# big-nacho/patolette

Measured on AMD Instinct MI355X. Metric: Mpixels/sec quantized (256-color ICtCp + KMeans) at 1 GPU; palette ΔE vs ref, higher is better.
Workload: dtype f64

## Files before the change

patolette_amd/csrc/pipeline.hip:

```cpp
#include <algorithm>
#include <functional>
#include <chrono>
#include <cmath>
#include <atomic>
#include <memory>
#include <mutex>
#include <thread>
#include <future>

#include "color_device.h"
#include "common.h"
#include "host_math.h"
#include "kmeans.h"
#include "map.h"
#include "saliency.h"
#include "quant.h"
#include "rgba.h"
#include "compact.h"

namespace pamd {

void launch_convert(int which, const double *src, double *dst, size_t n, ConvertStats *stats, hipStream_t s, BinK sumk = BinK{0.0, 0.0},
                    BinK momk = BinK{0.0, 0.0}, size_t begin = 0, size_t end = ~(size_t)0, bool init_stats = true);
void launch_convert_rows(int which, const double *rows, double *dst, size_t n, ConvertStats *stats, hipStream_t s,
// ... 124 lines not shown
    while (hi - lo > 1) { const int mid = (lo + hi) >> 1; if (t0[mid] <= t) lo = mid; else hi = mid; }
    return lo;
}
__global__ __launch_bounds__(256) void k_round_setup(NodeDev *table, RoundSetup a) {
    const size_t tid = (size_t)blockIdx.x * blockDim.x + threadIdx.x, stride = (size_t)gridDim.x * blockDim.x;
    for (size_t i = tid; i < (size_t)a.nr; i += stride) {
        const NodeIn in = a.recs[i];
        NodeDev &d = table[a.ids[i]];
        d.begin = in.begin; d.n = in.n; d.gn = in.gn; d.buf = in.buf; d.slot = in.slot; d.child0 = in.child0; d.nchild = in.nchild;
        for (int j = 0; j < 3; j++) { d.axis[j] = in.axis[j]; d.mean[j] = in.mean[j]; }
        d.sw = in.sw; d.klin = in.klin; d.kquad = in.kquad;
    }
    for (size_t i = tid; i < (size_t)a.nr * kNodeResetElems; i += stride)
        node_reset_element(table[a.ids[i / kNodeResetElems]], (int)(i % kNodeResetElems));
    for (size_t t = tid; t < (size_t)a.ntA; t += stride) {
        const int r = node_of_tile(a.tA0, a.nr, (int)t);
        const unsigned long long o = (unsigned long long)((int)t - a.tA0[r]) * kTileA, n = a.recs[r].n;
        a.tilesA[t] = Tile{a.recs[r].begin + o, (unsigned)(n - o < (unsigned long long)kTileA ? n - o : kTileA), (unsigned)a.ids[r]};
    }
    for (size_t t = tid; t < (size_t)a.ntP; t += stride) {
        const int r = node_of_tile(a.tP0, a.nr, (int)t);
        const unsigned long long o = (unsigned long long)((int)t - a.tP0[r]) * kTileP, n = a.recs[r].n;
        a.tilesP[t] = Tile{a.recs[r].begin + o, (unsigned)(n - o < (unsigned long long)kTileP ? n - o : kTileP), (unsigned)a.ids[r]};
    }
    for (size_t i = tid; i < a.nhist; i += stride) a.hist[i] = 0.0;
    for (size_t i = tid; i < a.nbk; i += stride) { a.hsize[i] = 0ULL; a.hcount[i] = 0u; }
}


struct GqOut { int kbase, error, pad[2]; int cuts[16]; unsigned long long ticks[8]; };

constexpr int kLqDevMaxK = 256;
constexpr int kLqNodeCap = 16 * kLqDevMaxK + 256;
constexpr int kLqRoundCap = 512;
constexpr int kLqMaxRounds = 96;

struct LqRec {
    double val;
    int left;
    int kn;
};
struct LqCen { double mean[3]; double gn; };
struct LqHead {
    int done, error, rounds, nnodes, neval, pad;
    unsigned long long split_evals, split_px;
    double tau;
    double round_px[kLqMaxRounds], round_nr[kLqMaxRounds];
};
struct LqCtl {
    LqHead h;
    int K, M, nleaves, pad;
    int ncids[2];
    RoundDyn dyn;
    int leaves[kLqNodeCap];
    int round_ids[kLqRoundCap];
    int cids[2][2 * kLqRoundCap];
    int tA0[kLqRoundCap + 1], tP0[kLqRoundCap + 1];
    int nparent[kLqNodeCap];
    double np[kLqNodeCap];
    LqRec nrec[kLqNodeCap];
    LqCen ncen[kLqNodeCap];
};
template <> struct WsPoison<LqCtl> {
    static void dev(LqCtl *p, size_t a, size_t b) {
        for (size_t i = a; i < b; i++) {
            char *c = reinterpret_cast<char *>(p + i);
            ws_poison_dev(c + offsetof(LqCtl, h) + offsetof(LqHead, tau), sizeof(double) * (1 + 2 * kLqMaxRounds));
            ws_poison_dev(c + offsetof(LqCtl, np), sizeof(LqCtl::np));
            ws_poison_dev_rows(c + offsetof(LqCtl, nrec), sizeof(LqRec), sizeof(double), kLqNodeCap);
            ws_poison_dev(c + offsetof(LqCtl, ncen), sizeof(LqCtl::ncen));
        }
    }
    static void host(LqCtl *, size_t, size_t) {}
};

template <int CTRL, int ROW_MASK>
__device__ __forceinline__ double dpp_max_f64(const double v) {
    const int lo = __double2loint(v), hi = __double2hiint(v);
    const int tlo = __builtin_amdgcn_update_dpp(lo, lo, CTRL, ROW_MASK, 0xf, false);
    const int thi = __builtin_amdgcn_update_dpp(hi, hi, CTRL, ROW_MASK, 0xf, false);
    return fmax(v, __hiloint2double(thi, tlo));
}

__global__ __launch_bounds__(256) void k_lq_children(NodeDev *nodes, LqCtl *c, const int call, int init_kbase,
                                                     const int init_first, int init_nnodes, const int init_K, const GqOut *gq) {
    const bool init = init_kbase > 0;
    if (!init && c->h.done) return;
    if (init && gq) { init_kbase = gq->kbase; init_nnodes = init_first + init_kbase; }
    const int ncids = init ? init_kbase : c->ncids[call & 1];
    const int wave = (int)blockIdx.x * 4 + (int)(threadIdx.x >> 6), lane = threadIdx.x & 63;
    if (init && blockIdx.x == 0 && threadIdx.x == 0) {
        c->K = init_K; c->M = init_K - init_kbase; c->nleaves = 0; c->ncids[0] = init_kbase; c->dyn = RoundDyn{0, 0, 0, 0};
        c->h.done = 0; c->h.error = 0; c->h.rounds = 0; c->h.nnodes = init_nnodes; c->h.neval = 0; c->h.split_evals = 0ULL; c->h.split_px = 0ULL;
        c->h.tau = 0.0;
        for (int r = 0; r < kLqMaxRounds; r++) { c->h.round_px[r] = 0.0; c->h.round_nr[r] = 0.0; }
        if (gq && gq->error) { c->h.done = 1; c->h.error = 3; c->ncids[0] = 0; }
        for (int i = 0; i < init_first; i++) { c->nrec[i] = LqRec{0.0, -1, 1}; c->np[i] = 0.0; c->nparent[i] = -1; }
    }
    if (init && gq && gq->error) return;
    if (wave >= ncids) return;
    const int id = init ? init_first + wave : c->cids[call & 1][wave];
    if (init && lane == 0) c->cids[0][wave] = id;
    NodeDev &d = nodes[id];
    const double *acc = &d.acc[0][0][0];
    double sum = 0;
    if (lane < 14) {
        double v[kSlots];
#pragma unroll
        for (int k = 0; k < kSlots; k++) v[k] = acc[k * 14 + lane];
#pragma unroll
        for (int k = 0; k < kSlots; k++) sum += v[k];
    }
    const double pair = sum + __shfl_down(sum, 1, 64);
    double cov[7];
#pragma unroll
    for (int q = 0; q < 7; q++)
        cov[q] = __hiloint2double(__builtin_amdgcn_readlane(__double2hiint(pair), 2 * q), __builtin_amdgcn_readlane(__double2loint(pair), 2 * q));
    if (lane != 0) return;
    double ub = cov[6];
    const bool single = d.gn <= 1ULL;
    const double sw = d.sw;
    if (single || !(sw > 0)) ub = 0;
    else {
        double c6[6];
        for (int q = 0; q < 6; q++) c6[q] = cov[q] / sw;
        const double b = hm::lambda_max_bound(c6) * sw * (1.0 + 1e-9) + 1e-9 * cov[6];
        if (b == b && b < ub) ub = b;
    }
    for (int q = 0; q < 6; q++) d.cov6[q] = cov[q];
    d.dist = cov[6]; d.ub = ub; d.axis_state = 0;
    c->nrec[id] = LqRec{single ? 0.0 : ub, -1, single ? 1 : 0};
    c->nparent[id] = init ? -1 : c->round_ids[wave >> 1];
    c->ncen[id] = LqCen{{d.mean[0], d.mean[1], d.mean[2]}, (double)d.gn};
    c->leaves[(init ? 0 : c->nleaves) + wave] = id;
}

__device__ __forceinline__ int block_excl_scan_256(const int v, int *sw , int &total) {
    const int lane = threadIdx.x & 63, wid = threadIdx.x >> 6;
    const int inc = (int)wave_scan_incl_u32((unsigned)v);
    __syncthreads();
    if (lane == 63) sw[wid] = inc;
    __syncthreads();
    int base = 0;
    for (int w = 0; w < wid; w++) base += sw[w];
    total = sw[0] + sw[1] + sw[2] + sw[3];
    return base + inc - v;
}

__device__ __forceinline__ unsigned long long lq_key(const double p) { return p > 0.0 ? (unsigned long long)__double_as_longlong(p) : 0ULL; }

constexpr double kSpecBeta = 0.25;

__global__ __launch_bounds__(256) void k_lq_select(NodeDev *nodes, LqCtl *c, const int call, const int e_lin, const int e_quad) {
    if (c->h.done) return;
    const int tid = threadIdx.x, lane = tid & 63;
    const int cur = call & 1, nxt = cur ^ 1;
    const int ncids = c->ncids[cur];
    if (blockIdx.x > 0) {
        const int w = ((int)blockIdx.x - 1) * 4 + (tid >> 6);
        if (w >= ncids) return;
        NodeDev &d = nodes[c->cids[cur][w]];
        if (d.gn <= 1ULL || !(d.sw > 0)) { if (lane == 0) d.axis_state = d.gn <= 1ULL ? 0 : -1; return; }
        double c6[6];
        for (int q = 0; q < 6; q++) c6[q] = d.cov6[q] / d.sw;
        double a[9] = {c6[0], c6[1], c6[2], c6[1], c6[3], c6[4], c6[2], c6[4], c6[5]};
        double wv[3];
        const int info = hm::eigen_sym3(a, wv);
        if (lane == 0) {
            if (info != 0) d.axis_state = -1;
            else { d.axis[0] = a[6]; d.axis[1] = a[7]; d.axis[2] = a[8]; d.axis_state = 1; }
        }
        return;
    }
    __shared__ int sw[5];
    __shared__ unsigned int hist[256];
    __shared__ unsigned long long s_prefix, s_px;
    __shared__ int s_need, s_neval, s_first;
    __shared__ double s_umax[4];
    const int M = c->M;
    const int nn = c->h.nnodes;
    const int nr_prev = c->dyn.nr;
    int evald = 0;
    for (int i = tid; i < nr_prev; i += 256) {
        const int id = c->round_ids[i];
        const NodeDev &d = nodes[id];
        if (d.axis_state < 0) { c->nrec[id] = LqRec{0.0, -1, 1}; c->np[id] = 0.0; continue; }
        const int l = d.child0;
        const double b = d.dist - (nodes[l].dist + nodes[l + 1].dist);
        const int par = c->nparent[id];
        const double pp = par < 0 ? INFINITY : c->np[par];
        c->nrec[id].val = b; c->nrec[id].kn = 1;
        c->np[id] = b < pp ? b : pp;
        evald++;
    }
    if (tid == 0) { s_neval = 0; s_px = 0ULL; }
    __syncthreads();
    if (evald) atomicAdd(&s_neval, evald);
    __syncthreads();
    const int neval = c->h.neval + s_neval;
    double tau = 0.0;
    if (neval >= M && M > 0) {
        unsigned long long prefix = 0ULL;
        int need = M;
        for (int pass = 0; pass < 3; pass++) {
            const int shift = 56 - 8 * pass;
            hist[tid] = 0u;
            __syncthreads();
            for (int i = tid; i < nn; i += 256) {
                const LqRec r = c->nrec[i];
                if (r.kn && r.left >= 0) {
                    const unsigned long long k = lq_key(c->np[i]);
                    if (pass == 0 || (k >> (shift + 8)) == (prefix >> (shift + 8))) atomicAdd(&hist[(k >> shift) & 255ULL], 1u);
                }
            }
            __syncthreads();
            {
                const int mine = (int)hist[255 - tid];
                int total;
                const int excl = block_excl_scan_256(mine, sw, total);
                if (tid == 0) s_first = 256;
                __syncthreads();
                if (excl + mine >= need && tid <= 254) atomicMin(&s_first, tid);
                __syncthreads();
                const int f = s_first;
                if (f < 256) { if (tid == f) { s_need = need - excl; s_prefix = prefix | ((unsigned long long)(255 - f) << shift); } }
                else if (tid == 254) { s_need = need - (excl + mine); s_prefix = prefix; }
            }
            __syncthreads();
            need = s_need; prefix = s_prefix;
        }
        tau = __longlong_as_double((long long)prefix);
    }
    const double thr = fmax(kDelta, tau * (1.0 - 1e-9));
    const int nleaves = c->nleaves + ncids;
    auto leaf_prio = [&](const int id) -> double {
        const LqRec r = c->nrec[id];
        const int par = c->nparent[id];
        if (r.kn || (par >= 0 && nodes[par].axis_state < 0)) return -1.0;
        const double pp = par < 0 ? INFINITY : c->np[par];
        return r.val < pp ? r.val : pp;
    };
    double thr2 = thr;
    if (c->h.rounds < 48) {
        double u = -1.0;
        for (int i = tid; i < nleaves; i += 256) { const double pr = leaf_prio(c->leaves[i]); u = pr > u ? pr : u; }
#pragma unroll
        for (int o = 32; o > 0; o >>= 1) { const double v = __shfl_xor(u, o, 64); u = v > u ? v : u; }
        __syncthreads();
        if (lane == 0) s_umax[tid >> 6] = u;
        __syncthreads();
        u = fmax(fmax(s_umax[0], s_umax[1]), fmax(s_umax[2], s_umax[3]));
        if (kSpecBeta * u > thr2) thr2 = kSpecBeta * u;
    }
    int nkeep = 0, nr = 0;
    for (int base = 0; base < nleaves; base += 256) {
        const int i = base + tid;
        int id = -1, sel = 0, keep = 0;
        if (i < nleaves) {
            id = c->leaves[i];
            const double pr = leaf_prio(id);
            sel = pr >= thr2 ? 1 : 0;
            keep = (!sel && pr >= thr) ? 1 : 0;
        }
        int tsel, tkeep;
        const int psel = block_excl_scan_256(sel, sw, tsel);
        if (nr + tsel > kLqRoundCap && sel && nr + psel >= kLqRoundCap) { sel = 0; keep = 1; }
        const int pkeep = block_excl_scan_256(keep, sw, tkeep);
        if (sel) c->round_ids[nr + psel] = id;
        __syncthreads();
        if (keep) c->leaves[nkeep + pkeep] = id;
        nr = min(nr + tsel, kLqRoundCap);
        nkeep += tkeep;
        __syncthreads();
    }
    if (nr == 0) {
        if (tid == 0) { c->h.done = 1; c->h.neval = neval; c->h.tau = tau; c->nleaves = 0; c->ncids[nxt] = 0; c->dyn = RoundDyn{0, 0, 0, 0}; }
        return;
    }
    if (nn + 2 * nr > kLqNodeCap) {
        if (tid == 0) { c->h.done = 1; c->h.error = 2; c->dyn = RoundDyn{0, 0, 0, 0}; }
        return;
    }
    int runA = 0, runP = 0;
    for (int base = 0; base < nr; base += 256) {
        const int r = base + tid;
        int ta = 0, tp = 0;
        unsigned long long n = 0ULL;
        if (r < nr) {
            const int id = c->round_ids[r];
            NodeDev &d = nodes[id];
            d.slot = r; d.child0 = nn + 2 * r; d.nchild = 2;
            int P = 1;
            while ((1ULL << P) < (d.gn > 1ULL ? d.gn : 2ULL)) P++;
            d.klin = make_bink(e_lin, P); d.kquad = make_bink(e_quad, P);
            c->nrec[id].left = nn + 2 * r;
            c->cids[nxt][2 * r] = nn + 2 * r; c->cids[nxt][2 * r + 1] = nn + 2 * r + 1;
            n = d.n;
            ta = (int)((n + kTileA - 1) / kTileA); tp = (int)((n + kTileP - 1) / kTileP);
        }
        int totA, totP;
        const int pa = block_excl_scan_256(ta, sw, totA);
        const int pp = block_excl_scan_256(tp, sw, totP);
        if (r < nr) { c->tA0[r] = runA + pa; c->tP0[r] = runP + pp; }
        runA += totA; runP += totP;
        for (int o = 32; o > 0; o >>= 1) n += __shfl_xor(n, o, 64);
        if (lane == 0 && n) atomicAdd(&s_px, n);
    }
    __syncthreads();
    if (tid == 0) {
        const int round = c->h.rounds;
        const unsigned long long rpx = s_px;
        c->tA0[nr] = runA; c->tP0[nr] = runP;
        c->nleaves = nkeep; c->ncids[nxt] = 2 * nr;
        c->dyn = RoundDyn{nr, runA, runP, 0};
        c->h.nnodes = nn + 2 * nr; c->h.neval = neval; c->h.tau = tau;
        c->h.split_evals += (unsigned long long)nr; c->h.split_px += rpx; c->h.rounds = round + 1;
        if (round < kLqMaxRounds) { c->h.round_px[round] = (double)rpx; c->h.round_nr[round] = (double)nr; }
    }
}

__global__ __launch_bounds__(256) void k_lq_export(const LqCtl *c, LqHead *head, LqRec *rec, LqCen *cen) {
    const int nn = c->h.nnodes;
    const int t = blockIdx.x * blockDim.x + threadIdx.x, stride = gridDim.x * blockDim.x;
    for (int i = t; i < nn; i += stride) { rec[i] = c->nrec[i]; cen[i] = c->ncen[i]; }
    const double *src = reinterpret_cast<const double *>(&c->h);
    double *dst = reinterpret_cast<double *>(head);
    for (int i = t; i < (int)(sizeof(LqHead) / sizeof(double)); i += stride) dst[i] = src[i];
}

struct LqCommit { int row, node, new_row, left; };
__global__ void k_lq_trace(const NodeDev *nodes, const LqCommit *commits, int n, patolette_amd__SplitRecord *out) {
    const int t = blockIdx.x * blockDim.x + threadIdx.x;
    if (t >= n) return;
    const LqCommit cm = commits[t];
    const NodeDev &h = nodes[cm.node], &hl = nodes[cm.left], &hr = nodes[cm.left + 1];
    patolette_amd__SplitRecord tr;
    tr.row = cm.row; tr.new_row = cm.new_row;
    tr.split = hl.psplit < 0 ? -1 : (hl.psplit & 0xffff); tr.degenerate = hl.psplit < 0 ? 0 : (hl.psplit >> 16) & 1;
    tr.n = h.gn; tr.n_left = hl.gn; tr.n_right = hr.gn; tr.sw = h.sw;
    for (int j = 0; j < 3; j++) tr.axis[j] = h.axis[j];
    for (int q = 0; q < 6; q++) tr.cov6[q] = h.cov6[q] / h.sw;
    tr.dist = h.dist; tr.dist_left = hl.dist; tr.dist_right = hr.dist; tr.benefit = h.dist - (hl.dist + hr.dist);
    out[t] = tr;
}

__global__ __launch_bounds__(256) void k_round_setup_dyn(NodeDev *table, const LqCtl *c, Tile *tilesA, Tile *tilesP, double *hist,
                                                         unsigned long long *hsize, unsigned int *hcount, const size_t lqs) {
    const int nr = c->dyn.nr;
    if (nr == 0) return;
    const int ntA = c->dyn.ntA, ntP = c->dyn.ntP;
    const size_t tid = (size_t)blockIdx.x * blockDim.x + threadIdx.x, stride = (size_t)gridDim.x * blockDim.x;
    for (size_t i = tid; i < (size_t)nr * kNodeResetElems; i += stride)
        node_reset_element(table[c->round_ids[i / kNodeResetElems]], (int)(i % kNodeResetElems));
    for (size_t t = tid; t < (size_t)ntA; t += stride) {
        const int r = node_of_tile(c->tA0, nr, (int)t);
        const NodeDev &d = table[c->round_ids[r]];
        const unsigned long long o = (unsigned long long)((int)t - c->tA0[r]) * kTileA, n = d.n;
        tilesA[t] = Tile{d.begin + o, (unsigned)(n - o < (unsigned long long)kTileA ? n - o : kTileA), (unsigned)c->round_ids[r]};
    }
    for (size_t t = tid; t < (size_t)ntP; t += stride) {
        const int r = node_of_tile(c->tP0, nr, (int)t);
        const NodeDev &d = table[c->round_ids[r]];
        const unsigned long long o = (unsigned long long)((int)t - c->tP0[r]) * kTileP, n = d.n;
        tilesP[t] = Tile{d.begin + o, (unsigned)(n - o < (unsigned long long)kTileP ? n - o : kTileP), (unsigned)c->round_ids[r]};
    }
    for (size_t i = tid; i < lqs * (size_t)nr; i += stride) hist[i] = 0.0;
    for (size_t i = tid; i < (size_t)nr * kBuckets; i += stride) { hsize[i] = 0ULL; hcount[i] = 0u; }
}

struct GqTab {
    unsigned long long w0[kBuckets + 1];
    double t[10][kBuckets + 9];
    __device__ double distortion(int a, int b) const {
        if (w0[a] == w0[b]) return 0;
        const double q0 = t[0][b] - t[0][a], q1 = t[1][b] - t[1][a], q2 = t[2][b] - t[2][a];
        return t[3][b] - t[3][a] - (q0 * q0 + q1 * q1 + q2 * q2) / (double)(w0[b] - w0[a]);
    }
    __device__ double vcov(int a, int b, int r, int s) const {
        if (w0[a] == w0[b]) return 0;
        const double cnt = (double)(w0[b] - w0[a]);
        const int rs = 4 + s * (s + 1) / 2 + r;
        return (t[rs][b] - t[rs][a]) / cnt - (t[r][b] - t[r][a]) * (t[s][b] - t[s][a]) / (cnt * cnt);
    }
    __device__ bool axis(int a, int b, double ax[3]) const {
        double m[9] = {0, 0, 0, 0, 0, 0, 0, 0, 0};
        for (int s = 0; s < 3; s++) for (int r = 0; r <= s; r++) m[s * 3 + r] = vcov(a, b, r, s);
        m[0 * 3 + 2] = m[2 * 3 + 0]; m[0 * 3 + 1] = m[1 * 3 + 0]; m[1 * 3 + 2] = m[2 * 3 + 1];
        double w[3];
        if (hm::eigen_sym3(m, w) != 0) return false;
        ax[0] = m[6]; ax[1] = m[7]; ax[2] = m[8];
        return true;
    }
    __device__ static double norm3(const double a[3]) { double s = 0; for (int i = 0; i < 3; i++) s += a[i] * a[i]; return sqrt(s); }
    __device__ double bias(int a, int b, const double ax[3]) const {
        double ca[3];
        if (!axis(a, b, ca)) return -1;
        const double norms = norm3(ax) * norm3(ca);
        if (norms < 1e-16) return 0;
        const double dot = (ca[0] * ax[0] + ca[1] * ax[1] + ca[2] * ax[2]);
        return fmin(1.0, fabs(dot / norms));
    }
};

__device__ __forceinline__ void gq_dp_entry(const GqTab &c, const double *Ep, const int k, const int n, const int lane, double &e_out, int &cut_out) {
    double best = INFINITY; int bt = -1;
    for (int t = n - 2 - lane; t >= k - 1; t -= 64) {
        const double v = Ep[t] + c.distortion(t, n);
        if (v < best) { best = v; bt = t; }
    }
#pragma unroll
    for (int o = 32; o > 0; o >>= 1) {
        const double v2 = __shfl_down(best, o, 64); const int t2 = __shfl_down(bt, o, 64);
        if (t2 >= 0 && (bt < 0 || v2 < best || (v2 == best && t2 > bt))) { best = v2; bt = t2; }
    }
    double e = Ep[n - 1]; int cut = n - 1;
    if (bt >= 0 && best < e) { e = best; cut = bt; }
    e_out = e; cut_out = cut;
}

__global__ __launch_bounds__(1024) void k_gq_control(const double *__restrict__ hist, const unsigned int *__restrict__ hcount, GqDpDev *g,
                                                     const int palette_size, const int weighted, NodeDev *nodes, const int base0,
                                                     unsigned char *lut, GqOut *out, GqOut *out_host) {
    __shared__ GqTab c;
    __shared__ double E[2][kBuckets + 1];
    __shared__ int s_q[16], s_nq, s_stop, s_err, s_top;
    __shared__ double s_ax[3], s_cd[16], s_cb[16];
    __shared__ unsigned char s_lut[kBuckets];
    __shared__ double s_part[kGqMaxK][4][2];
    __shared__ unsigned long long s_cnt[kGqMaxK];
    const int tid = threadIdx.x, lane = tid & 63, wv = tid >> 6;
    __shared__ unsigned long long s_ticks[8];
    if (tid == 0) { for (int i = 0; i < 8; i++) s_ticks[i] = 0; s_ticks[0] = wall_clock64(); }
    for (int i = tid; i < 10 * kBuckets; i += 1024) {
        const int hq = i / kBuckets, b = i - hq * kBuckets;
        c.t[hq][b + 1] = hist[(size_t)(hq * 2 + 0) * kBuckets + b] + hist[(size_t)(hq * 2 + 1) * kBuckets + b];
    }
    for (int b = tid; b < kBuckets; b += 1024) c.w0[b + 1] = hcount[b];
    if (tid < 10) c.t[tid][0] = 0;
    if (tid == 10) c.w0[0] = 0;
    __syncthreads();
    if (tid == 0) s_ticks[5] = wall_clock64();
    if (wv < 10) {
        double *t = c.t[wv];
        double v[8];
#pragma unroll
        for (int u = 0; u < 8; u++) v[u] = t[1 + lane * 8 + u];
        double carry = 0, cin = 0;
        for (int l = 0; l < 64; l++) {
            double a = carry;
#pragma unroll
// ... 200 lines not shown
    if (i >= n) return;
    NodeDev &d = table[ids[i]];
    for (int q = 0; q < 7; q++) {
        for (int k = 1; k < kSlots; k++) { d.acc[k][q][0] = 0; d.acc[k][q][1] = 0; }
        d.acc[0][q][0] = buf[(size_t)i * 14 + 2 * q]; d.acc[0][q][1] = buf[(size_t)i * 14 + 2 * q + 1];
    }
}
__global__ void k_shard_children_local(NodeDev *table, const int *round_nodes, int nround) {
    const int i = blockIdx.x * blockDim.x + threadIdx.x;
    if (i >= nround) return;
    const NodeDev &nd = table[round_nodes[i]];
    for (int k = 0; k < nd.nchild; k++) {
        NodeDev &ch = table[nd.child0 + k];
        ch.begin = nd.cbegin[k]; ch.n = nd.cbegin[k + 1] - nd.cbegin[k];
    }
}

struct Bounds {
    double cmax, range, wmax; int e_lin, e_quad; double lo[3], hi[3];
    bool have_sum = false; double sum[3] = {0, 0, 0};
    bool have_mom = false;
    double sum2[3][2] = {{0, 0}, {0, 0}, {0, 0}}, mom2[6][2] = {{0, 0}, {0, 0}, {0, 0}, {0, 0}, {0, 0}, {0, 0}};
    bool nonfinite = false;
};

static int exp_bound(double v) {
    if (!(v > 0) || !std::isfinite(v)) return 1;
    return std::ilogb(v) + 1;
}

struct Shard {
    size_t total = 0, begin = 0;
    patolette_amd__Comm comm{};
};

struct Engine {
    int device = -1;
    hipStream_t stream = nullptr;
    const Shard *shard = nullptr;
    bool invariant = false;
    DevBuf<unsigned char> commbuf;
    PinBuf<unsigned char> h_comm;
    DevBuf<int> shard_ids;
    PinBuf<float> h_cent;
    PinBuf<ConvertStats> h_cstats;
    hipEvent_t ev_stats = nullptr;
    hipStream_t stream2 = nullptr;
    hipEvent_t ev_up[2] = {nullptr, nullptr}, ev_join = nullptr;
    size_t prep_N = 0, prep_planes = 0;
    DevBuf<double> src, wsrc, cvt, bufA, bufB, aux;
    DevBuf<unsigned short> bkt;
    DevBuf<NodeDev> nodes;
    DevBuf<NodeIn> stage_in;
    DevBuf<NodeOut> stage_out;
    DevBuf<int> ids, round_nodes, node_tile0;
    DevBuf<Tile> tilesA, tilesP;
    DevBuf<double> hist, sum6, dpal;
    DevBuf<unsigned long long> hsize, tileoff;
    DevBuf<unsigned int> hcount, tilecnt;
    DevBuf<unsigned char> lut, dmap, src8, pal8, quant8;
    DevBuf<unsigned> rgba_cnt;
    DevBuf<int> rgba_cpos;
    DevBuf<unsigned char> rgba_rgb, rgba_map;
    DevBuf<double> rgba_w;
    PinBuf<unsigned> h_rgba_m;
    DevBuf<ConvertStats> cstats;
    PinBuf<NodeIn> h_stage_in;
    PinBuf<NodeOut> h_stage_out;
    PinBuf<int> h_ids, h_ids_get;
    PinBuf<Tile> h_tilesA, h_tilesP;
    PinBuf<int> h_round, h_tile0;
    PinBuf<double> h_dbl;
    PinBuf<unsigned char> h_bytes, h_packet, h_mapstage;
    DevBuf<unsigned char> packet;
    KMeansWork km;
    NNWork nn;
    SalWork sal;
    DevBuf<double> wsal;
    DevBuf<GqDpDev> gq;
    PinBuf<GqDpDev> h_gq;
    DevBuf<GqOut> gqout;
    PinBuf<GqOut> h_gqout;
    PinBuf<double> h_pal;
    DevBuf<LqCtl> lqctl;
    PinBuf<LqHead> h_lqhead;
    PinBuf<LqRec> h_lqrec;
    PinBuf<LqCen> h_lqcen;
    std::vector<LqRec> lq_rec_local;
    std::vector<LqCommit> lq_commits;
    bool trace_pending = false;
    size_t lq_hint_N = 0, lq_hint_K = 0; int lq_hint_rounds = 0;
    DevBuf<int> perm_dev;
    size_t perm_N = 0, perm_nx = 0;
    PinBuf<int32_t> h_perm;
    size_t hperm_N = 0, hperm_nx = 0;
    hm::PermScratch perm_ws;
    std::future<void> perm_job;
    patolette_amd__Stats stats{};
    double ms_saliency = 0.0;
    std::string last_error;
    std::vector<double> map_palette;
    patolette_amd__SplitTrace trace_hdr{};
    std::vector<patolette_amd__SplitRecord> trace;
    std::vector<double> cluster_centers;

    void init() {
        if (stream) return;
        int cnt = 0;
        if (hipGetDeviceCount(&cnt) != hipSuccess || cnt <= 0)
            throw HipError("patolette_amd: no HIP device available (this library has no CPU fallback)");
        if (device < 0) { HIP_CHECK(hipGetDevice(&device)); }
        HIP_CHECK(hipSetDevice(device));
        HIP_CHECK(hipStreamCreateWithFlags(&stream, hipStreamNonBlocking));
    }
    void sync() { HIP_CHECK(hipStreamSynchronize(stream)); if (ktimer().enabled) ktimer().collect(); }
    ~Engine() {
        if (stream) { (void)hipSetDevice(device); (void)hipStreamSynchronize(stream); if (ev_stats) (void)hipEventDestroy(ev_stats);
                      for (hipEvent_t e : {ev_up[0], ev_up[1], ev_join}) if (e) (void)hipEventDestroy(e);
                      if (stream2) (void)hipStreamDestroy(stream2);
                      (void)hipStreamDestroy(stream); }
    }
};

namespace {
std::mutex g_pool_mu;
std::vector<Engine *> g_pool;
thread_local int tl_invariant = -1;
bool invariant_default() {
    static const bool env = getenv("PAMD_INVARIANT_SUMS") && atoi(getenv("PAMD_INVARIANT_SUMS")) != 0;
    return tl_invariant < 0 ? env : tl_invariant != 0;
}
Engine *pool_acquire(int device, bool invariant) {
    {
        std::lock_guard<std::mutex> lk(g_pool_mu);
        for (size_t i = 0; i < g_pool.size(); i++)
            if (g_pool[i]->device == device || g_pool[i]->device < 0) {
                Engine *e = g_pool[i];
                g_pool.erase(g_pool.begin() + i);
                if (e->device < 0) e->device = device;
                e->invariant = invariant;
                return e;
            }
    }
    Engine *e = new Engine;
    e->device = device;
    e->invariant = invariant;
    return e;
}
void pool_release(Engine *e) { std::lock_guard<std::mutex> lk(g_pool_mu); g_pool.push_back(e); }
struct EngineHolder {
    Engine *e = nullptr;
    ~EngineHolder() { if (e) pool_release(e); }
};
EngineHolder &holder() { static thread_local EngineHolder h; return h; }
}

static Engine &engine() {
    EngineHolder &h = holder();
    if (!h.e) {
        int dev = -1;
        if (hipGetDevice(&dev) != hipSuccess) dev = -1;
        h.e = pool_acquire(dev, invariant_default());
    }
    return *h.e;
}

// ... 233 lines not shown
                int second = -1; double sv = -1;
                for (size_t j = 0; j < count; j++) if ((int)j != best && fkn[j] && fval[j] > sv) { sv = fval[j]; second = (int)j; }
                if (second >= 0 && sv >= kDelta && sv < bv) { best = second; bv = sv; }
            }
            if (!(bv >= kDelta)) { out.stopped_early = true; break; }
            const int id = result[best], l = rec[id].left;
            out.commits.push_back(LqCommit{best, id, (int)count, l});
            result[count] = l; result[best] = l + 1;
            fval[count] = rec[l].val; fkn[count] = (char)rec[l].kn;
            fval[best] = rec[l + 1].val; fkn[best] = (char)rec[l + 1].kn;
            count++;
            continue;
        }
        if (std::max(best >= 0 ? bv : 0.0, mu) < kDelta) { out.stopped_early = true; break; }
        return false;
    }
    result.resize(count);
    return true;
}

static bool lq_replay(const LqRec *rec, int kbase, int first_base, size_t K, LqReplay &out) {
    std::vector<int> &result = out.result;
    result.assign(K, -1);
    for (int j = 0; j < kbase; j++) result[j] = first_base + j;
    size_t count = (size_t)kbase;
    constexpr size_t B = 16;
    const size_t nb = (K + B - 1) / B;
    std::vector<double> fval(nb * B, 0.0);
    std::vector<char> fkn(nb * B, 0);
    std::vector<double> bbv(nb, 0.0), bmu(nb, -1.0);
    std::vector<int> bbest(nb, -1);
    auto rescan = [&](const size_t b) {
        int best = -1; double bv = 0, mu = -1;
        const size_t lo = b * B, hi = std::min(count, lo + B);
        for (size_t j = lo; j < hi; j++) {
            if (fkn[j]) { if (best < 0 || fval[j] > bv) { bv = fval[j]; best = (int)j; } }
            else if (fval[j] > mu) mu = fval[j];
        }
        bbest[b] = best; bbv[b] = bv; bmu[b] = mu;
    };
    for (size_t j = 0; j < count; j++) { fval[j] = rec[result[j]].val; fkn[j] = (char)rec[result[j]].kn; }
    for (size_t b = 0; b < nb; b++) rescan(b);
    const int fault = g_debug_fault.load(std::memory_order_relaxed);
    while (count < K) {
        int best = -1; double bv = 0, mu = -1;
        const size_t nbu = (count + B - 1) / B;
        for (size_t b = 0; b < nbu; b++) {
            if (bbest[b] >= 0 && (best < 0 || bbv[b] > bv)) { bv = bbv[b]; best = bbest[b]; }
            if (bmu[b] > mu) mu = bmu[b];
        }
        if (mu < 0 || (best >= 0 && bv > mu)) {
            if (fault == 2) {
                int second = -1; double sv = -1;
                for (size_t j = 0; j < count; j++) if ((int)j != best && fkn[j] && fval[j] > sv) { sv = fval[j]; second = (int)j; }
                if (second >= 0 && sv >= kDelta && sv < bv) { best = second; bv = sv; }
            }
            if (!(bv >= kDelta)) { out.stopped_early = true; break; }
            const int id = result[best], l = rec[id].left;
            out.commits.push_back(LqCommit{best, id, (int)count, l});
            result[count] = l; result[best] = l + 1;
            fval[count] = rec[l].val; fkn[count] = (char)rec[l].kn;
            fval[best] = rec[l + 1].val; fkn[best] = (char)rec[l + 1].kn;
            count++;
            rescan((size_t)best / B);
            if ((count - 1) / B != (size_t)best / B) rescan((count - 1) / B);
            continue;
        }
        if (std::max(best >= 0 ? bv : 0.0, mu) < kDelta) { out.stopped_early = true; break; }
        return false;
    }
    result.resize(count);
    return true;
}

std::atomic<int> g_lq_device{getenv("PAMD_LQ_DEVICE") ? atoi(getenv("PAMD_LQ_DEVICE")) : 2};
std::atomic<int> g_gq_device{getenv("PAMD_GQ_DEVICE") ? atoi(getenv("PAMD_GQ_DEVICE")) : 1};
constexpr size_t kLqDeviceAutoPixels = (size_t)40 << 20;

static bool lq_device_eligible(const Engine &E, size_t N, size_t K, bool verbose, bool allow_device) {
    const int lq_mode = g_lq_device.load(std::memory_order_relaxed);
    return allow_device && (lq_mode == 1 || (lq_mode == 2 && N < kLqDeviceAutoPixels)) && !E.shard && !verbose && K <= (size_t)kLqDevMaxK;
}

static void ws_prepare(Engine &E, size_t N, size_t K, bool weighted, bool verbose) {
    const size_t planes = weighted ? 4 : 3;
    const bool lq_dev = lq_device_eligible(E, N, K, verbose, true);
    const size_t slack = lq_dev ? (size_t)kLqRoundCap : 0, ntA = ceil_div(N, (size_t)kTileA) + slack, ntP = ceil_div(N, (size_t)kTileP) + slack;
    const size_t tables = lq_dev ? (size_t)kLqRoundCap * kBuckets : (size_t)kBuckets;
    E.cvt.reserve(planes * N); E.cstats.reserve(1);
    E.bufA.reserve(planes * N + 64); E.bufB.reserve(planes * N + 64); E.bkt.reserve(N);
    E.tilesA.reserve(ntA); E.tilesP.reserve(ntP);
    E.tilecnt.reserve(ntP * kMaxChildren); E.tileoff.reserve(ntP * kMaxChildren);
    E.round_nodes.reserve(1); E.node_tile0.reserve(2); E.h_round.reserve(kBuckets);
    E.hist.reserve(std::max(hist_slot_doubles(), lq_dev ? (size_t)kNQ_LQ * 2 * kBuckets * kLqRoundCap : 0));
    E.hsize.reserve(tables); E.hcount.reserve(tables); E.lut.reserve(tables);
    E.nodes.reserve(std::max<size_t>(4 * K + 64, lq_dev ? (size_t)kLqNodeCap : 0));
    E.h_dbl.reserve(16 * kBuckets * 2 + 64);
    E.gq.reserve(1); E.gqout.reserve(1); E.h_gqout.reserve(1); E.h_gq.reserve(1);
    const size_t nput = kGqMaxK + 1;
    E.stage_in.reserve(nput); E.stage_out.reserve(nput); E.ids.reserve(nput); E.h_stage_in.reserve(nput); E.h_stage_out.reserve(nput);
    E.h_ids.reserve(nput); E.h_ids_get.reserve(nput);
    E.h_cent.reserve(3 * K);
    if (lq_dev) { E.lqctl.reserve(1); E.h_lqhead.reserve(1); E.h_lqrec.reserve(kLqNodeCap); E.h_lqcen.reserve(kLqNodeCap); }
}

static int lq_device_loop(Engine &E, size_t N, size_t K, bool weighted, bool inv_sums, const Bounds &bnd, const QuantBuffers &qlq, int kbase,
                          int first_base, int nnodes, std::vector<double> &centers, size_t &len, unsigned long long *max_members) {
    hipStream_t s = E.stream;
    const size_t lqs = (size_t)kNQ_LQ * 2 * kBuckets;
    const int ntA_ub = (int)ceil_div(N, (size_t)kTileA) + kLqRoundCap, ntP_ub = (int)ceil_div(N, (size_t)kTileP) + kLqRoundCap;
    E.lqctl.reserve(1); E.h_lqhead.reserve(1); E.h_lqrec.reserve(kLqNodeCap); E.h_lqcen.reserve(kLqNodeCap);
    E.hist.reserve(std::max(hist_slot_doubles(), lqs * kLqRoundCap)); E.hsize.reserve((size_t)kLqRoundCap * kBuckets);
    E.hcount.reserve((size_t)kLqRoundCap * kBuckets); E.lut.reserve((size_t)kLqRoundCap * kBuckets);
    E.tilesA.reserve(ntA_ub); E.tilesP.reserve(ntP_ub);
    E.tilecnt.reserve((size_t)ntP_ub * kMaxChildren); E.tileoff.reserve((size_t)ntP_ub * kMaxChildren);
    LqCtl *c = E.lqctl.p;
    LqHead *head = E.h_lqhead.p;
    for (int r = 0; r < kLqMaxRounds; r++) { head->round_px[r] = 0.0; head->round_nr[r] = 0.0; }
    const RoundDyn *dyn = &c->dyn;
    const int *d_round = c->round_ids, *d_tP0 = c->tP0;
    int call = 0;
    const GqOut *gq = kbase < 0 ? (const GqOut *)E.gqout.p : nullptr;
    const int kb_ub = kbase < 0 ? kGqMaxK : kbase;
    auto control = [&]() {
        const bool first = call == 0;
        {
            KTIME("k_lq_children", s, 0.0);
            if (first) hipLaunchKernelGGL(k_lq_children, (kb_ub + 3) / 4, 256, 0, s, E.nodes.p, c, call, kb_ub, first_base, nnodes, (int)K, gq);
            else hipLaunchKernelGGL(k_lq_children, 2 * kLqRoundCap / 4, 256, 0, s, E.nodes.p, c, call, 0, 0, 0, 0, (const GqOut *)nullptr);
        }
        KTIME("k_lq_select", s, 0.0);
        hipLaunchKernelGGL(k_lq_select, 1 + (first ? (kb_ub + 3) / 4 : 2 * kLqRoundCap / 4), 256, 0, s, E.nodes.p, c, call, bnd.e_lin, bnd.e_quad);
        HIP_CHECK(hipGetLastError());
        call++;
    };
    int enq = 0;
    auto round = [&]() {
        if (enq >= kLqMaxRounds) throw HipError("patolette_amd: split loop exceeded its round limit");
        const double *px_src = &head->round_px[enq], *nr_src = &head->round_nr[enq];
        const bool rev = enq % 2 == 1;
        static const bool setup_kernel = getenv("PAMD_LQ_SETUP_KERNEL") && atoi(getenv("PAMD_LQ_SETUP_KERNEL")) != 0;
        if (setup_kernel) {
            hipLaunchKernelGGL(k_round_setup_dyn, 1024, 256, 0, s, E.nodes.p, (const LqCtl *)c, E.tilesA.p, E.tilesP.p, E.hist.p, E.hsize.p, E.hcount.p, lqs);
            HIP_CHECK(hipGetLastError());
            launch_minmax(qlq, E.tilesA.p, ntA_ub, 0, E.nodes.p, s, rev, dyn, px_src);
        } else {
            const RoundLists rl{c->round_ids, c->tA0, c->tP0, E.tilesA.p, E.tilesP.p, E.hist.p, lqs, E.hsize.p, E.hcount.p};
            launch_minmax(qlq, E.tilesA.p, ntA_ub, 0, E.nodes.p, s, rev, dyn, px_src, &rl);
        }
        launch_hist(qlq, false, E.tilesA.p, ntA_ub, 0, E.nodes.p, E.hist.p, E.hsize.p, E.hcount.p, s, !rev, false, dyn, px_src);
        launch_cut(weighted, E.nodes.p, d_round, kLqRoundCap, E.hist.p, E.hsize.p, E.hcount.p, E.lut.p, s, dyn, nr_src);
        launch_partition(qlq, E.tilesP.p, ntP_ub, 0, d_round, d_tP0, kLqRoundCap, E.nodes.p, E.lut.p, E.tilecnt.p, E.tileoff.p, true, s, inv_sums, rev, dyn, px_src);
        enq++;
        control();
    };
    control();
    int want = (E.lq_hint_N == N && E.lq_hint_K == K && E.lq_hint_rounds > 0) ? E.lq_hint_rounds : 9;
    const bool fault_full = g_debug_fault.load(std::memory_order_relaxed) == 4;
    if (fault_full) want = 3;
    for (;;) {
        while (enq < want) round();
        hipLaunchKernelGGL(k_lq_export, 16, 256, 0, s, (const LqCtl *)c, head, E.h_lqrec.p, E.h_lqcen.p);
        HIP_CHECK(hipGetLastError());
        E.sync();
        if (fault_full) return -2;
        if (head->done) break;
        want = enq + 2;
    }
    if (head->error == 2) return -2;
    if (head->error == 3) return -1;
    if (kbase < 0) kbase = E.h_gqout.p->kbase;
    E.lq_hint_N = N; E.lq_hint_K = K; E.lq_hint_rounds = head->rounds;
    LqReplay rp;
    const double t_rp0 = now_ms();
    E.lq_rec_local.resize((size_t)head->nnodes);
    std::memcpy(E.lq_rec_local.data(), E.h_lqrec.p, (size_t)head->nnodes * sizeof(LqRec));
    const bool replay_ok = lq_replay(E.lq_rec_local.data(), kbase, first_base, K, rp);
    const double t_rp1 = now_ms();
    static const bool replay_check = getenv("PAMD_LQ_REPLAY_CHECK") != nullptr;
    if (replay_check || !replay_ok) {
        LqReplay ref;
        const bool ref_ok = lq_replay_plain(E.lq_rec_local.data(), kbase, first_base, K, ref);
        if (ref_ok != replay_ok || ref.result != rp.result || ref.stopped_early != rp.stopped_early)
            fprintf(stderr, "patolette_amd: split loop: the two replays DISAGREE (plain %d, %zu rows; blocked %d, %zu rows), kbase %d, K %zu, nodes %d, rounds %d\n",
                    (int)ref_ok, ref.result.size(), (int)replay_ok, rp.result.size(), kbase, K, head->nnodes, head->rounds);
        else if (!replay_ok)
            fprintf(stderr, "patolette_amd: split loop: both replays blocked after %zu commits, kbase %d, K %zu, nodes %d, rounds %d, evaluated %d, tau %.17g\n",
                    rp.commits.size(), kbase, K, head->nnodes, head->rounds, head->neval, head->tau);
    }
    if (!replay_ok) throw HipError("patolette_amd: split loop: the replay met an unevaluated node");
    len = rp.result.size();
    centers.assign(3 * len, 0.0);
    unsigned long long mg = 0;
    for (size_t i = 0; i < len; i++) {
        const LqCen &cn = E.h_lqcen.p[rp.result[i]];
        for (int j = 0; j < 3; j++) centers[(size_t)j * len + i] = cn.mean[j];
        mg = std::max(mg, (unsigned long long)cn.gn);
    }
    if (max_members) *max_members = mg;
    E.stats.split_evals = (size_t)head->split_evals; E.stats.split_px = (size_t)head->split_px; E.stats.lq_rounds = (size_t)head->rounds;
    E.lq_commits.swap(rp.commits);
    E.trace.clear();
    E.trace_pending = true;
    E.trace_hdr.stopped_early = rp.stopped_early ? 1 : 0;
    static const bool lq_times = getenv("PAMD_LQ_TIMES") != nullptr;
    if (lq_times) {
        fprintf(stderr, "patolette_amd: device-driven split loop: %d rounds, %d evaluated, %zu commits, tau %.3g; host replay %.1f us\n", head->rounds, head->neval,
                E.lq_commits.size(), head->tau, 1e3 * (t_rp1 - t_rp0));
        if (gq) {
            const unsigned long long *t = E.h_gqout.p->ticks;
            fprintf(stderr, "patolette_amd: k_gq_control us: prefixes %.1f, axis %.1f, search %.1f, records %.1f\n", (t[1] - t[0]) * 0.01, (t[2] - t[1]) * 0.01,
                    (t[3] - t[2]) * 0.01, (t[4] - t[3]) * 0.01);
            fprintf(stderr, "patolette_amd: k_gq_control us: of the prefixes, staging %.1f\n", (t[5] - t[0]) * 0.01);
        }
    }
    return 0;
}

static void materialise_trace(Engine &E) {
    if (!E.trace_pending) return;
    E.trace_pending = false;
    const int n = (int)E.lq_commits.size();
    E.trace.assign(n, patolette_amd__SplitRecord{});
    if (!n) return;
    DevBuf<LqCommit> dc; DevBuf<patolette_amd__SplitRecord> dr;
    dc.reserve(n); dr.reserve(n);
    HIP_CHECK(hipMemcpyAsync(dc.p, E.lq_commits.data(), sizeof(LqCommit) * n, hipMemcpyHostToDevice, E.stream));
    hipLaunchKernelGGL(k_lq_trace, (n + 63) / 64, 64, 0, E.stream, (const NodeDev *)E.nodes.p, (const LqCommit *)dc.p, n, dr.p);
    HIP_CHECK(hipGetLastError());
    HIP_CHECK(hipMemcpyAsync(E.trace.data(), dr.p, sizeof(patolette_amd__SplitRecord) * n, hipMemcpyDeviceToHost, E.stream));
    HIP_CHECK(hipStreamSynchronize(E.stream));
}
// ... 1782 lines not shown
```

Measured before the change: 3091.

## Fuse per-round LQ children and select kernels into one ticketed control kernel

For every round after the first, the separate k_lq_children and k_lq_select launches are replaced by one k_lq_control kernel. Half of its blocks compute the child sums and eigen axes redundantly. The other half compute bounds and records, then take an atomic ticket so the last-arriving block runs the serial select step. This removes one kernel launch and its dependency gap per split round. The cost is the duplicated child-sum work, reliance on relaxed atomics, fences and a last-block pattern for cross-block visibility, and a ticket counter that must be reset correctly. The unused env-gated setup kernel path is also removed.

Result: no change. 3107, median of 6 (+0.5%).

```diff
diff --git a/patolette_amd/csrc/pipeline.hip b/patolette_amd/csrc/pipeline.hip
--- a/patolette_amd/csrc/pipeline.hip
+++ b/patolette_amd/csrc/pipeline.hip
@@ -230,6 +230,49 @@
     return fmax(v, __hiloint2double(thi, tlo));
 }
 
+__device__ __forceinline__ void lq_child_sums(const NodeDev &d, const int lane, double (&cov)[7]) {
+    const double *acc = &d.acc[0][0][0];
+    double sum = 0;
+    if (lane < 14) {
+        double v[kSlots];
+#pragma unroll
+        for (int k = 0; k < kSlots; k++) v[k] = acc[k * 14 + lane];
+#pragma unroll
+        for (int k = 0; k < kSlots; k++) sum += v[k];
+    }
+    const double pair = sum + __shfl_down(sum, 1, 64);
+#pragma unroll
+    for (int q = 0; q < 7; q++)
+        cov[q] = __hiloint2double(__builtin_amdgcn_readlane(__double2hiint(pair), 2 * q), __builtin_amdgcn_readlane(__double2loint(pair), 2 * q));
+}
+__device__ __forceinline__ double lq_child_bound(const NodeDev &d, const double (&cov)[7]) {
+    double ub = cov[6];
+    const double sw = d.sw;
+    if (d.gn <= 1ULL || !(sw > 0)) ub = 0;
+    else {
+        double c6[6];
+        for (int q = 0; q < 6; q++) c6[q] = cov[q] / sw;
+        const double b = hm::lambda_max_bound(c6) * sw * (1.0 + 1e-9) + 1e-9 * cov[6];
+        if (b == b && b < ub) ub = b;
+    }
+    return ub;
+}
+__device__ __forceinline__ void lq_child_axis(NodeDev &d, const int lane, const double *cov6) {
+    if (d.gn <= 1ULL || !(d.sw > 0)) { if (lane == 0) __hip_atomic_store(&d.axis_state, d.gn <= 1ULL ? 0 : -1, __ATOMIC_RELAXED, __HIP_MEMORY_SCOPE_AGENT); return; }
+    double c6[6];
+    for (int q = 0; q < 6; q++) c6[q] = cov6[q] / d.sw;
+    double a[9] = {c6[0], c6[1], c6[2], c6[1], c6[3], c6[4], c6[2], c6[4], c6[5]};
+    double wv[3];
+    const int info = hm::eigen_sym3(a, wv);
+    if (lane == 0) {
+        if (info != 0) __hip_atomic_store(&d.axis_state, -1, __ATOMIC_RELAXED, __HIP_MEMORY_SCOPE_AGENT);
+        else {
+            for (int j = 0; j < 3; j++) __hip_atomic_store(&d.axis[j], a[6 + j], __ATOMIC_RELAXED, __HIP_MEMORY_SCOPE_AGENT);
+            __hip_atomic_store(&d.axis_state, 1, __ATOMIC_RELAXED, __HIP_MEMORY_SCOPE_AGENT);
+        }
+    }
+}
+
 __global__ __launch_bounds__(256) void k_lq_children(NodeDev *nodes, LqCtl *c, const int call, int init_kbase,
                                                      const int init_first, int init_nnodes, const int init_K, const GqOut *gq) {
     const bool init = init_kbase > 0;
@@ -250,31 +293,11 @@
     const int id = init ? init_first + wave : c->cids[call & 1][wave];
     if (init && lane == 0) c->cids[0][wave] = id;
     NodeDev &d = nodes[id];
-    const double *acc = &d.acc[0][0][0];
-    double sum = 0;
-    if (lane < 14) {
-        double v[kSlots];
-#pragma unroll
-        for (int k = 0; k < kSlots; k++) v[k] = acc[k * 14 + lane];
-#pragma unroll
-        for (int k = 0; k < kSlots; k++) sum += v[k];
-    }
-    const double pair = sum + __shfl_down(sum, 1, 64);
     double cov[7];
-#pragma unroll
-    for (int q = 0; q < 7; q++)
-        cov[q] = __hiloint2double(__builtin_amdgcn_readlane(__double2hiint(pair), 2 * q), __builtin_amdgcn_readlane(__double2loint(pair), 2 * q));
+    lq_child_sums(d, lane, cov);
     if (lane != 0) return;
-    double ub = cov[6];
     const bool single = d.gn <= 1ULL;
-    const double sw = d.sw;
-    if (single || !(sw > 0)) ub = 0;
-    else {
-        double c6[6];
-        for (int q = 0; q < 6; q++) c6[q] = cov[q] / sw;
-        const double b = hm::lambda_max_bound(c6) * sw * (1.0 + 1e-9) + 1e-9 * cov[6];
-        if (b == b && b < ub) ub = b;
-    }
+    const double ub = lq_child_bound(d, cov);
     for (int q = 0; q < 6; q++) d.cov6[q] = cov[q];
     d.dist = cov[6]; d.ub = ub; d.axis_state = 0;
     c->nrec[id] = LqRec{single ? 0.0 : ub, -1, single ? 1 : 0};
@@ -299,27 +322,10 @@
 
 constexpr double kSpecBeta = 0.25;
 
-__global__ __launch_bounds__(256) void k_lq_select(NodeDev *nodes, LqCtl *c, const int call, const int e_lin, const int e_quad) {
-    if (c->h.done) return;
+__device__ __forceinline__ void lq_select_block(NodeDev *nodes, LqCtl *c, const int call, const int e_lin, const int e_quad) {
     const int tid = threadIdx.x, lane = tid & 63;
     const int cur = call & 1, nxt = cur ^ 1;
     const int ncids = c->ncids[cur];
-    if (blockIdx.x > 0) {
-        const int w = ((int)blockIdx.x - 1) * 4 + (tid >> 6);
-        if (w >= ncids) return;
-        NodeDev &d = nodes[c->cids[cur][w]];
-        if (d.gn <= 1ULL || !(d.sw > 0)) { if (lane == 0) d.axis_state = d.gn <= 1ULL ? 0 : -1; return; }
-        double c6[6];
-        for (int q = 0; q < 6; q++) c6[q] = d.cov6[q] / d.sw;
-        double a[9] = {c6[0], c6[1], c6[2], c6[1], c6[3], c6[4], c6[2], c6[4], c6[5]};
-        double wv[3];
-        const int info = hm::eigen_sym3(a, wv);
-        if (lane == 0) {
-            if (info != 0) d.axis_state = -1;
-            else { d.axis[0] = a[6]; d.axis[1] = a[7]; d.axis[2] = a[8]; d.axis_state = 1; }
-        }
-        return;
-    }
     __shared__ int sw[5];
     __shared__ unsigned int hist[256];
     __shared__ unsigned long long s_prefix, s_px;
@@ -467,6 +473,69 @@
     }
 }
 
+__global__ __launch_bounds__(256) void k_lq_select(NodeDev *nodes, LqCtl *c, const int call, const int e_lin, const int e_quad) {
+    if (c->h.done) return;
+    if (blockIdx.x > 0) {
+        const int w = ((int)blockIdx.x - 1) * 4 + (int)(threadIdx.x >> 6);
+        if (w >= c->ncids[call & 1]) return;
+        NodeDev &d = nodes[c->cids[call & 1][w]];
+        lq_child_axis(d, threadIdx.x & 63, d.cov6);
+        return;
+    }
+    lq_select_block(nodes, c, call, e_lin, e_quad);
+}
+
+__global__ __launch_bounds__(256) void k_lq_control(NodeDev *nodes, LqCtl *c, const int call, const int e_lin, const int e_quad, unsigned int *ticket) {
+    if (c->h.done) return;
+    const int lane = threadIdx.x & 63, half = (int)gridDim.x / 2;
+    const int cur = call & 1, ncids = c->ncids[cur];
+    const bool solver = (int)blockIdx.x >= half;
+    const int wave = ((int)blockIdx.x - (solver ? half : 0)) * 4 + (int)(threadIdx.x >> 6);
+    if (((int)blockIdx.x - (solver ? half : 0)) * 4 >= ncids) return;
+    if (solver) {
+        if (wave >= ncids) return;
+        NodeDev &d = nodes[c->cids[cur][wave]];
+        double cov[7];
+        lq_child_sums(d, lane, cov);
+        lq_child_axis(d, lane, cov);
+        return;
+    }
+    __shared__ int s_last;
+    if (wave < ncids) {
+        const int id = c->cids[cur][wave];
+        NodeDev &d = nodes[id];
+        double cov[7];
+        lq_child_sums(d, lane, cov);
+        if (lane == 0) {
+            const bool single = d.gn <= 1ULL;
+            const double ub = lq_child_bound(d, cov);
+            for (int q = 0; q < 6; q++) d.cov6[q] = cov[q];
+            d.ub = ub;
+            c->ncen[id] = LqCen{{d.mean[0], d.mean[1], d.mean[2]}, (double)d.gn};
+            __hip_atomic_store(&d.dist, cov[6], __ATOMIC_RELAXED, __HIP_MEMORY_SCOPE_AGENT);
+            __hip_atomic_store(&c->nrec[id].val, single ? 0.0 : ub, __ATOMIC_RELAXED, __HIP_MEMORY_SCOPE_AGENT);
+            __hip_atomic_store(&c->nrec[id].left, -1, __ATOMIC_RELAXED, __HIP_MEMORY_SCOPE_AGENT);
+            __hip_atomic_store(&c->nrec[id].kn, single ? 1 : 0, __ATOMIC_RELAXED, __HIP_MEMORY_SCOPE_AGENT);
+            __hip_atomic_store(&c->nparent[id], c->round_ids[wave >> 1], __ATOMIC_RELAXED, __HIP_MEMORY_SCOPE_AGENT);
+            __hip_atomic_store(&c->leaves[c->nleaves + wave], id, __ATOMIC_RELAXED, __HIP_MEMORY_SCOPE_AGENT);
+            asm volatile("s_waitcnt vmcnt(0)" ::: "memory");
+        }
+    }
+    __syncthreads();
+    if (threadIdx.x == 0) {
+        const unsigned tk = __hip_atomic_fetch_add(ticket, 1u, __ATOMIC_RELAXED, __HIP_MEMORY_SCOPE_AGENT);
+        const bool last = tk == (unsigned)((ncids + 3) / 4) - 1u;
+        if (last) {
+            __hip_atomic_store(ticket, 0u, __ATOMIC_RELAXED, __HIP_MEMORY_SCOPE_AGENT);
+            __builtin_amdgcn_fence(__ATOMIC_ACQUIRE, "agent");
+            asm volatile("s_waitcnt vmcnt(0)" ::: "memory");
+        }
+        s_last = last ? 1 : 0;
+    }
+    __syncthreads();
+    if (s_last) lq_select_block(nodes, c, call, e_lin, e_quad);
+}
+
 __global__ __launch_bounds__(256) void k_lq_export(const LqCtl *c, LqHead *head, LqRec *rec, LqCen *cen) {
     const int nn = c->h.nnodes;
     const int t = blockIdx.x * blockDim.x + threadIdx.x, stride = gridDim.x * blockDim.x;
@@ -490,30 +559,6 @@
     for (int q = 0; q < 6; q++) tr.cov6[q] = h.cov6[q] / h.sw;
     tr.dist = h.dist; tr.dist_left = hl.dist; tr.dist_right = hr.dist; tr.benefit = h.dist - (hl.dist + hr.dist);
     out[t] = tr;
-}
-
-__global__ __launch_bounds__(256) void k_round_setup_dyn(NodeDev *table, const LqCtl *c, Tile *tilesA, Tile *tilesP, double *hist,
-                                                         unsigned long long *hsize, unsigned int *hcount, const size_t lqs) {
-    const int nr = c->dyn.nr;
-    if (nr == 0) return;
-    const int ntA = c->dyn.ntA, ntP = c->dyn.ntP;
-    const size_t tid = (size_t)blockIdx.x * blockDim.x + threadIdx.x, stride = (size_t)gridDim.x * blockDim.x;
-    for (size_t i = tid; i < (size_t)nr * kNodeResetElems; i += stride)
-        node_reset_element(table[c->round_ids[i / kNodeResetElems]], (int)(i % kNodeResetElems));
-    for (size_t t = tid; t < (size_t)ntA; t += stride) {
-        const int r = node_of_tile(c->tA0, nr, (int)t);
-        const NodeDev &d = table[c->round_ids[r]];
-        const unsigned long long o = (unsigned long long)((int)t - c->tA0[r]) * kTileA, n = d.n;
-        tilesA[t] = Tile{d.begin + o, (unsigned)(n - o < (unsigned long long)kTileA ? n - o : kTileA), (unsigned)c->round_ids[r]};
-    }
-    for (size_t t = tid; t < (size_t)ntP; t += stride) {
-        const int r = node_of_tile(c->tP0, nr, (int)t);
-        const NodeDev &d = table[c->round_ids[r]];
-        const unsigned long long o = (unsigned long long)((int)t - c->tP0[r]) * kTileP, n = d.n;
-        tilesP[t] = Tile{d.begin + o, (unsigned)(n - o < (unsigned long long)kTileP ? n - o : kTileP), (unsigned)c->round_ids[r]};
-    }
-    for (size_t i = tid; i < lqs * (size_t)nr; i += stride) hist[i] = 0.0;
-    for (size_t i = tid; i < (size_t)nr * kBuckets; i += stride) { hsize[i] = 0ULL; hcount[i] = 0u; }
 }
 
 struct GqTab {
@@ -880,6 +925,7 @@
     DevBuf<GqOut> gqout;
     PinBuf<GqOut> h_gqout;
     PinBuf<double> h_pal;
+    DevBuf<unsigned int> lqtick;
     DevBuf<LqCtl> lqctl;
     PinBuf<LqHead> h_lqhead;
     PinBuf<LqRec> h_lqrec;
@@ -1279,6 +1325,12 @@
     return allow_device && (lq_mode == 1 || (lq_mode == 2 && N < kLqDeviceAutoPixels)) && !E.shard && !verbose && K <= (size_t)kLqDevMaxK;
 }
 
+static void lq_tick_reserve(Engine &E) {
+    const size_t n = 32;
+    if (E.lqtick.cap >= n) return;
+    E.lqtick.reserve(n);
+    HIP_CHECK(hipMemsetAsync(E.lqtick.p, 0, n * sizeof(unsigned int), E.stream));
+}
 static void ws_prepare(Engine &E, size_t N, size_t K, bool weighted, bool verbose) {
     const size_t planes = weighted ? 4 : 3;
     const bool lq_dev = lq_device_eligible(E, N, K, verbose, true);
@@ -1298,7 +1350,7 @@
     E.stage_in.reserve(nput); E.stage_out.reserve(nput); E.ids.reserve(nput); E.h_stage_in.reserve(nput); E.h_stage_out.reserve(nput);
     E.h_ids.reserve(nput); E.h_ids_get.reserve(nput);
     E.h_cent.reserve(3 * K);
-    if (lq_dev) { E.lqctl.reserve(1); E.h_lqhead.reserve(1); E.h_lqrec.reserve(kLqNodeCap); E.h_lqcen.reserve(kLqNodeCap); }
+    if (lq_dev) { E.lqctl.reserve(1); E.h_lqhead.reserve(1); E.h_lqrec.reserve(kLqNodeCap); E.h_lqcen.reserve(kLqNodeCap); lq_tick_reserve(E); }
 }
 
 static int lq_device_loop(Engine &E, size_t N, size_t K, bool weighted, bool inv_sums, const Bounds &bnd, const QuantBuffers &qlq, int kbase,
@@ -1306,7 +1358,7 @@
     hipStream_t s = E.stream;
     const size_t lqs = (size_t)kNQ_LQ * 2 * kBuckets;
     const int ntA_ub = (int)ceil_div(N, (size_t)kTileA) + kLqRoundCap, ntP_ub = (int)ceil_div(N, (size_t)kTileP) + kLqRoundCap;
-    E.lqctl.reserve(1); E.h_lqhead.reserve(1); E.h_lqrec.reserve(kLqNodeCap); E.h_lqcen.reserve(kLqNodeCap);
+    E.lqctl.reserve(1); E.h_lqhead.reserve(1); E.h_lqrec.reserve(kLqNodeCap); E.h_lqcen.reserve(kLqNodeCap); lq_tick_reserve(E);
     E.hist.reserve(std::max(hist_slot_doubles(), lqs * kLqRoundCap)); E.hsize.reserve((size_t)kLqRoundCap * kBuckets);
     E.hcount.reserve((size_t)kLqRoundCap * kBuckets); E.lut.reserve((size_t)kLqRoundCap * kBuckets);
     E.tilesA.reserve(ntA_ub); E.tilesP.reserve(ntP_ub);
@@ -1320,14 +1372,16 @@
     const GqOut *gq = kbase < 0 ? (const GqOut *)E.gqout.p : nullptr;
     const int kb_ub = kbase < 0 ? kGqMaxK : kbase;
     auto control = [&]() {
-        const bool first = call == 0;
-        {
-            KTIME("k_lq_children", s, 0.0);
-            if (first) hipLaunchKernelGGL(k_lq_children, (kb_ub + 3) / 4, 256, 0, s, E.nodes.p, c, call, kb_ub, first_base, nnodes, (int)K, gq);
-            else hipLaunchKernelGGL(k_lq_children, 2 * kLqRoundCap / 4, 256, 0, s, E.nodes.p, c, call, 0, 0, 0, 0, (const GqOut *)nullptr);
-        }
-        KTIME("k_lq_select", s, 0.0);
-        hipLaunchKernelGGL(k_lq_select, 1 + (first ? (kb_ub + 3) / 4 : 2 * kLqRoundCap / 4), 256, 0, s, E.nodes.p, c, call, bnd.e_lin, bnd.e_quad);
+        if (call == 0) {
+            { KTIME("k_lq_children", s, 0.0);
+              hipLaunchKernelGGL(k_lq_children, (kb_ub + 3) / 4, 256, 0, s, E.nodes.p, c, call, kb_ub, first_base, nnodes, (int)K, gq); }
+            KTIME("k_lq_select", s, 0.0);
+            hipLaunchKernelGGL(k_lq_select, 1 + (kb_ub + 3) / 4, 256, 0, s, E.nodes.p, c, call, bnd.e_lin, bnd.e_quad);
+        } else {
+            KTIME("k_lq_control", s, 0.0);
+            hipLaunchKernelGGL(k_lq_control, 2 * (2 * kLqRoundCap / 4), 256, 0, s, E.nodes.p, c, call, bnd.e_lin, bnd.e_quad,
+                               E.lqtick.p);
+        }
         HIP_CHECK(hipGetLastError());
         call++;
     };
@@ -1336,15 +1390,8 @@
         if (enq >= kLqMaxRounds) throw HipError("patolette_amd: split loop exceeded its round limit");
         const double *px_src = &head->round_px[enq], *nr_src = &head->round_nr[enq];
         const bool rev = enq % 2 == 1;
-        static const bool setup_kernel = getenv("PAMD_LQ_SETUP_KERNEL") && atoi(getenv("PAMD_LQ_SETUP_KERNEL")) != 0;
-        if (setup_kernel) {
-            hipLaunchKernelGGL(k_round_setup_dyn, 1024, 256, 0, s, E.nodes.p, (const LqCtl *)c, E.tilesA.p, E.tilesP.p, E.hist.p, E.hsize.p, E.hcount.p, lqs);
-            HIP_CHECK(hipGetLastError());
-            launch_minmax(qlq, E.tilesA.p, ntA_ub, 0, E.nodes.p, s, rev, dyn, px_src);
-        } else {
-            const RoundLists rl{c->round_ids, c->tA0, c->tP0, E.tilesA.p, E.tilesP.p, E.hist.p, lqs, E.hsize.p, E.hcount.p};
-            launch_minmax(qlq, E.tilesA.p, ntA_ub, 0, E.nodes.p, s, rev, dyn, px_src, &rl);
-        }
+        const RoundLists rl{c->round_ids, c->tA0, c->tP0, E.tilesA.p, E.tilesP.p, E.hist.p, lqs, E.hsize.p, E.hcount.p};
+        launch_minmax(qlq, E.tilesA.p, ntA_ub, 0, E.nodes.p, s, rev, dyn, px_src, &rl);
         launch_hist(qlq, false, E.tilesA.p, ntA_ub, 0, E.nodes.p, E.hist.p, E.hsize.p, E.hcount.p, s, !rev, false, dyn, px_src);
         launch_cut(weighted, E.nodes.p, d_round, kLqRoundCap, E.hist.p, E.hsize.p, E.hcount.p, E.lut.p, s, dyn, nr_src);
         launch_partition(qlq, E.tilesP.p, ntP_ub, 0, d_round, d_tP0, kLqRoundCap, E.nodes.p, E.lut.p, E.tilecnt.p, E.tileoff.p, true, s, inv_sums, rev, dyn, px_src);
```
